# thomasdeppisch/eMagLS

Measured on AMD Instinct MI355X. Metric: eMagLS filter sets/s (N=4, 2702 dirs, 512 taps), higher is better.
Workload: dtype f64; 1 GPU; BASELINE config 3: getEMagLsFilters em32 r=4.2cm N=4 complex-SH, 2702 dirs, 512 taps, 48 kHz; one filter set per step, inputs resident in HBM; dirs=2702, taps=512, sim_order=19, bins=512, k_cut=43, designs_resident_per_gpu=128, designs_per_batch=32, batches_in_flight=4, distinct_hrir_sets_resident=20, parallelism=independent jobs per GPU, one RCCL gather

## Files before the change

emagls_amd/csrc/args.hpp:

```cpp
#pragma once
#include "common.hpp"

namespace emagls {

struct FactorArgs {
    int S;
    int C;
    int ldS;
    int kb0;
    int P;
    const void* Tn;
    const cplx* bn;
    int nOrders;
    int bn_stride;
    const cplx* Xd;
    int64_t xd_stride;
    int reg_mode;
    double reg_c;
    double tol_dim;
    cplx* Z;
    cplx* Vws;
    double* sv;
    const cplx* Hq;
    int64_t ldHq;
// ... 50 lines not shown
    long long* timing;
    int fetch_mode;
    long long wait_ticks;
    int force_global;
    const double* dir_azi;
    const double* dir_zen;
    const double* mic_azi;
    const double* mic_zen;
    const int* smap;
    const cplx* bsc;
    int nord_pad;
    int synth_split;
    int synth_prio;
    const cplx* Winit;
    cplx* U;
};
constexpr int SWEEP_MULTI_MAX = 16;
struct HalfSweepMulti {
    int n;
    HalfSweepArgs a[SWEEP_MULTI_MAX];
};
constexpr int REG_SWEEP_MAX = 32;


}
```

emagls_amd/csrc/batch_run.hip:

```cpp
#include "host_internal.hpp"

void emagls_batch_forget(emagls_batch* b, emagls_plan* p) {
    for (auto& q : b->plans) if (q == p) q = nullptr;
}

namespace {
void batch_sweep_stage(emagls_batch& b) {
    const int nb = (int)b.plans.size();
    std::vector<HalfSweepArgs> ha((size_t)nb);
    for (int j = 0; j < nb; ++j) ha[j] = emagls_half_args(*b.plans[j]);
    if (b.atf_share || b.geo_share)
        for (int j = 1; j < nb; ++j) {
            ha[j].G = ha[0].G; ha[j].Yri = ha[0].Yri; ha[j].Mw = ha[0].Mw; ha[j].cond_ok = ha[0].cond_ok;
            ha[j].bsc = ha[0].bsc; ha[j].smap = ha[0].smap;
            ha[j].skip_flag = ha[0].skip_flag;
        }
    const bool reg = b.plans[0]->sweep_persist && reg_sweep_wanted(b.plans.data(), nb);
    for (auto* q : b.plans) q->reg_sweep = reg;
    if (!reg && nb > SWEEP_MULTI_MAX) throw Error(EMAGLS_ERR_UNSUPPORTED, "internal: more than 16 designs in a batch need the register-resident sweep");
    HalfSweepMulti h{};
    h.n = std::min(nb, SWEEP_MULTI_MAX);
    for (int j = 0; j < h.n; ++j) h.a[j] = ha[j];
    emagls_plan& q0 = *b.plans[0];
    const int kk0 = std::max(q0.kcut0, 1);
    if (kk0 >= q0.P) return;
    if (q0.sweep_persist) {
        hipStream_t ss = b.stream;
        {
            SweepGate gate(ss, reg ? reg_sweep_gate_cost((int)q0.D, nb) : 0);
            if (b.lanes) { BatchScope sc(nb, b.stride); launch_zero(q0.get("ll"), q0.bufs["ll"].bytes, ss); }
            else for (auto* q : b.plans) launch_zero(q->get("ll"), q->bufs["ll"].bytes, ss);
            if (reg) {
// ... 289 lines not shown
            };
            if (hh_end > 1) {
                bc("Yc", 0, g.bufs["Yc"].bytes);
                bc(cb ? "R" : "Rc", 0, g.bufs[cb ? "R" : "Rc"].bytes);
                bc("Vws", 0, sizeof(cplx) * (size_t)(hh_end - 1) * g.C * ldSh);
                bc("Nw", 0, sizeof(cplx) * (size_t)(hh_end - 1) * g.C * g.C);
                bc("tauw", 0, sizeof(double) * (size_t)(hh_end - 1) * g.C);
                bc("cond_ok", 0, sizeof(double) * (size_t)g.P);
            }
            if (gf > 0 && gf < ls_end) {
                bc("G", (size_t)(gf - g.g0) * g_stride_b, (size_t)(ls_end - gf) * g_stride_b);
                bc("Mw", 0, sizeof(cplx) * (size_t)ls_end * g.C * g.C);
            }
        }
        if (b.geo_ls_shared) geo_yls_stage(b, b.stream);
        hrir_side(1);
    } else if (b.lanes) {
        BatchScope sc(n, b.stride);
        Scoped from(p0.geo_from, &p0);
        emagls_post_sweep(p0);
    } else {
        for (auto* p : b.plans) {
            Scoped from(p->geo_from, &p0);
            emagls_post_sweep(*p);
        }
    }
}
void batch_execute_geo(emagls_batch& b) {
    const bool warm = batch_geo_next_is_warm(b);
    if (!warm) {
        b.geo_kept_version = ~0ull;
        b.geo_ran_version = batch_geo_version(b);
        b.geo_cold_pending = true;
        if (b.geo_ls_shared) {
            const emagls_plan& p0 = *b.plans[0];
            const int ls_end = std::min(p0.kcut0, p0.P), hh_ls = std::min(p0.hh_end, ls_end);
            const void *y0 = b.yls.get(), *z0 = b.zls.get();
            b.yls.grow(sizeof(cplx) * (size_t)(ls_end - 1) * p0.C * p0.ldD);
            b.zls.grow(sizeof(cplx) * (size_t)std::max(hh_ls, 1) * p0.C * p0.ldS_h);
            if (b.yls.get() != y0 || b.zls.get() != z0) { b.group[0].reset(); b.warm.reset(); }
        }
    }
    batch_run_two_graphs(b, warm ? b.warm : b.group[0], batch_geo_stage, warm ? 1 : 0, sweep_launch_count(*b.plans[0]));
    b.last_form = warm ? 2 : 1;
    ++(warm ? b.geo_warm_runs : b.geo_cold_runs);
}

void batch_magls_decide_sharing(emagls_batch& b, bool sweep_needed) {
    bool share = false;
    emagls_plan& p0 = *b.plans[0];
    if (b.geo_want && b.plans.size() > 1 && !p0.custom_basis && !p0.diffuse && (p0.sweep_persist || !sweep_needed)) {
        share = batch_inputs_same(b, {"hrir_azi", "hrir_zen"}, b.geo_checked_version, b.geo_inputs_same);
        for (auto* p : b.plans) share = share && !p->custom_basis && p->d.fs == p0.d.fs;
    }
    batch_set_sharing(b, b.geo_share, share);
// ... 287 lines not shown
```

emagls_amd/csrc/capi.hip:

```cpp
#include "host_internal.hpp"

namespace {

struct CachedPlan {
    std::unique_ptr<emagls_plan> plan;
    emagls_design_desc desc{};
    int device = 0;
    bool busy = false;
    uint64_t last_use = 0;
};
std::mutex g_cache_mu;
std::vector<CachedPlan> g_cache;
uint64_t g_cache_tick = 0;

int one_shot(const emagls_design_desc& desc, const double* hL, const double* hR, const double* azi, const double* zen,
             const double* mic_azi, const double* mic_zen, const double* atf, const double* atf_azi, const double* atf_zen,
             void* wL, void* wR, double* mean_dev, const void* Y_hrir = nullptr, const void* Y_mic = nullptr) {
    return guarded([&] {
        int dev = 0;
        HIP_CHECK(hipGetDevice(&dev));
        emagls_plan* p = nullptr;
        std::unique_ptr<emagls_plan> fresh;
        bool cached = false;
        {
// ... 436 lines not shown
    return guarded([&] {
        DeviceGuard dg(p ? p->device : -1);
        if (!p || !name || !nbytes) throw Error(EMAGLS_ERR_ARG, "null pointer");
        if (std::string(name) == "Yls") {
            emagls_batch* b = p->owner;
            if (!b || !b->geo_share || !b->geo_ls_shared || !b->yls.get()) throw Error(EMAGLS_ERR_ARG, "Yls: the plan's batch keeps no such operand");
            const emagls_plan& p0 = *b->plans[0];
            const size_t bytes = sizeof(cplx) * (size_t)(std::min(p0.kcut0, p0.P) - 1) * p0.C * p0.ldD;
            if (!dst) { *nbytes = bytes; return; }
            HIP_CHECK(hipStreamSynchronize(b->stream));
            const size_t n = std::min(*nbytes, bytes);
            HIP_CHECK(hipMemcpy(dst, b->yls.get(), n, hipMemcpyDeviceToHost));
            *nbytes = n;
            return;
        }
        auto it = p->bufs.find(name);
        if (it == p->bufs.end()) throw Error(EMAGLS_ERR_ARG, std::string("unknown buffer ") + name);
        if (!dst) { *nbytes = it->second.bytes; return; }
        HIP_CHECK(hipStreamSynchronize(p->stream));
        const size_t n = std::min(*nbytes, it->second.bytes);
        HIP_CHECK(hipMemcpy(dst, it->second.p, n, hipMemcpyDeviceToHost));
        *nbytes = n;
    });
}
void* emagls_plan_stream(emagls_plan* p) { return p ? (void*)p->stream : nullptr; }

int emagls_batch_create(emagls_plan** plans, int nplans, emagls_batch** batch) {
    return guarded([&] {
        if (!plans || !batch || nplans < 1) throw Error(EMAGLS_ERR_ARG, "invalid argument");
        const int batch_max = std::max(g_batch_max.load(), g_batch_max_override);
// ... 387 lines not shown
```

emagls_amd/csrc/device_mem.hpp:

```cpp
#pragma once
#include <hipfft/hipfft.h>

#include <algorithm>
#include <deque>

#include "kernels.hpp"

namespace emagls {

struct DevMem {
    DevMem() = default;
    explicit DevMem(size_t bytes) { alloc(bytes); }
    DevMem(DevMem&& o) noexcept : p_(o.p_), cap_(o.cap_) { o.p_ = nullptr; o.cap_ = 0; }
    DevMem& operator=(DevMem&& o) noexcept {
        if (this != &o) { reset(); p_ = o.p_; cap_ = o.cap_; o.p_ = nullptr; o.cap_ = 0; }
        return *this;
    }
    ~DevMem() { reset(); }
    void reset() {
        if (p_) (void)hipFree(p_);
        p_ = nullptr; cap_ = 0;
    }
    void alloc(size_t bytes) {
        reset();
        HIP_CHECK(hipMalloc(&p_, bytes));
        cap_ = bytes;
    }
    void grow(size_t bytes) {
        bytes = std::max<size_t>(bytes, 16);
        if (bytes > cap_) alloc(bytes);
    }
    template <typename T = void> T* get() const { return static_cast<T*>(p_); }
    size_t capacity() const { return cap_; }

private:
    void* p_ = nullptr;
    size_t cap_ = 0;
};

struct FftPlan {
    FftPlan() = default;
    FftPlan(FftPlan&& o) noexcept : h_(o.h_) { o.h_ = 0; }
    FftPlan& operator=(FftPlan&& o) noexcept {
        if (this != &o) { reset(); h_ = o.h_; o.h_ = 0; }
        return *this;
// ... 40 lines not shown
```

emagls_amd/csrc/host_internal.hpp:

```cpp
#pragma once
#include <atomic>
#include <chrono>
#include <cstdlib>
#include <cstring>
#include <deque>
#include <map>
#include <memory>
#include <mutex>
#include <shared_mutex>
#include <string>
#include <thread>
#include <utility>
#include <vector>

#include "../../include/emagls.h"
#include "array_model.hpp"
#include "device_mem.hpp"
#include "kernels.hpp"

using namespace emagls;

struct emagls_batch;
void emagls_batch_forget(emagls_batch* b, emagls_plan* p);

// ... 328 lines not shown
    hipStream_t stream = nullptr;
    bool own_stream = true;
    bool atf = false, atf_share = false, atf_inputs_same = false;
    uint64_t atf_checked_version = ~0ull;
    bool magls = false;
    bool geo_want = false, geo_share = false, geo_inputs_same = false;
    uint64_t geo_checked_version = ~0ull;
    uint64_t geo_kept_version = ~0ull;
    uint64_t geo_ran_version = ~0ull;
    bool geo_cold_pending = false;
    CapturedGraph warm;
    int last_form = 0;
    long long geo_cold_runs = 0, geo_warm_runs = 0;
    bool geo_ls_shared = false;
    emagls::DevMem yls, zls;
    emagls::DevMem cmp_flag;
    int nstreams = 1;
    hipStream_t side[3] = {nullptr, nullptr, nullptr};
    CapturedGraph group[4];
    int prof_level = 0;
    hipEvent_t sweep_ev[2] = {nullptr, nullptr};
    CapturedGraph post;
    bool side0_external = false;
    int order_hint = 0;
    int groups = 1;
    CapturedGraph group_hh[4];
    hipStream_t hh_stream[4] = {nullptr, nullptr, nullptr, nullptr};
    bool defer_hh = false;
    bool alone = true;
    int eager_runs = 0;
// ... 108 lines not shown
```

emagls_amd/csrc/kernels.hpp:

```cpp
#pragma once
#include <algorithm>
#include <functional>

#include "common.hpp"

namespace emagls {

void launch_zero(void* p, size_t bytes, hipStream_t st);
void launch_compare_words(const void* a, const void* b, size_t bytes, int* differ, hipStream_t st);
void launch_broadcast_lanes(const void* src, size_t bytes, size_t stride, int nlanes, hipStream_t st);
struct LanePtrs { void* p[64]; };
void launch_scatter_lanes(const void* srcL, const void* srcR, size_t stride, size_t bytes, int n, const LanePtrs& dst, hipStream_t st);
void launch_gather_buffers(const LanePtrs& src, const LanePtrs& dst, int nbuf, size_t bytes, hipStream_t st);
struct BufferMoves { const void* src[96]; void* dst[96]; size_t bytes[96]; int n; };
void launch_move_buffers(const BufferMoves& m, hipStream_t st);
void launch_ch_basis(int N, int M, const double* azi, bool cplx_basis, void* out, int ld, hipStream_t st, bool out_real = false);
void launch_sh_coeff(int N, double* tab, hipStream_t st);
inline size_t esz(bool c) { return c ? sizeof(cplx) : sizeof(double); }
inline size_t sh_coeff_count(int N) { return (size_t)2 * (N + 1) * (N + 1) + 2 * (N + 1); }
void launch_sh_basis(int N, int64_t D, const double* azi, const double* zen, const double* tab, bool cplx_basis,
                     void* Y, int64_t ld, hipStream_t st);
void launch_transpose_conj(const void* Y, int64_t D, int64_t S, int64_t ldY, void* Yt, int64_t Dpad, int64_t ldYt,
                           bool is_cplx, bool conj_it, hipStream_t st);

// ... 79 lines not shown
void launch_sweep_synth(const HalfSweepMulti& m, hipStream_t st);
void launch_yls_gram(const void* bsc, int nord_pad, const double* dir_azi, const double* dir_zen, const double* mic_azi, const double* mic_zen,
                     const int* smap, const double* Pm, const void* Mw, int D, int nOut, int kb_lo, int kb_hi, void* Yls, int64_t ldD, hipStream_t st);
void launch_ls_shared_rows(const void* Hc, int64_t ldH, int ls_end, const void* Yls, int64_t ldD, int D, int C, int P, void* W, hipStream_t st);
void synth_cosines_debug(const double* dir_azi, const double* dir_zen, int64_t ndirs, const double* mic_azi, const double* mic_zen, int nmics, double* x2);
void synth_operand_debug(const void* bsc, int nbins, int nord_pad, const double* x, int64_t nx, int gs, void* g_plus, void* g_minus);
int reg_sweep_max_units();
bool reg_sweep_supported(int D, int nmics, int nunits, int nOrd);
size_t reg_sweep_ll_bytes(int D, int nmics);
int reg_sweep_capacity(int D);
int reg_sweep_slots_per_xcd();
int reg_sweep_pick_waves(int D, int ndesigns);
int reg_sweep_gate_cost(int D, int ndesigns);
bool reg_sweep_fits(int D, int nmics, int nunits, int nOrd, int ndesigns);
void launch_sweep_reg(const HalfSweepArgs* args_dev, const HalfSweepArgs& a0, int n, hipStream_t st);
double reg_contract_selftest();
double gram_tile_selftest(bool four);
void store_sweep_args(const HalfSweepArgs* host, int n, HalfSweepArgs* dev, hipStream_t st);
void launch_sweep_finalize(const void* Wpart, void* W, int nWG, int C, int P, int kb_last, hipStream_t st);
void launch_hy_conj(const void* Hc, int64_t ldD, int nrows, const void* Yc, int64_t ldY, bool y_cplx, int D, int S, void* Pw, void* out,
                    int ldS, hipStream_t st);
size_t hy_workspace_elems(int nrows, int ldS);
void launch_ypinv(const void* Q, int64_t ldQ, bool q_cplx, const void* Zb, int ldS, int D, int S, int C, void* Ypinv,
                  int64_t ldD, hipStream_t st);
void launch_ls_apply(const void* Hc, int64_t ldH, int n_c, const void* Zf, bool z_cplx, int64_t ldD, int D, int C, int P,
                     int kb_lo, int kb_hi, void* W, hipStream_t st);
void launch_ls_filters(const double* hL, const double* hR, int64_t L, int D, const void* Yp, bool cplx_basis, int64_t ldD,
                       int C, void* wL, void* wR, hipStream_t st);
void launch_conj_copy(const void* in, void* out, int64_t n, bool is_cplx, hipStream_t st);
void launch_sh_rows_to_complex(void* W, int C, int nrows, int order, hipStream_t st);
// ... 201 lines not shown
```

emagls_amd/csrc/sweep_reg.hip:

```cpp
#include "device_mem.hpp"
#include "persist_common.hpp"
#include "synth_common.hpp"

#include <algorithm>
#include <map>
#include <mutex>

namespace emagls {

namespace {

constexpr int RG_MLD = 36;

constexpr int DPP_ROR4 = 0x124, DPP_ROR8 = 0x128;
__device__ __forceinline__ int rg_slot_set(int i, int x) { return i < 4 ? 0 : i < 8 ? 1 : x >> 1; }
__device__ __forceinline__ int rg_slot_unit(int i, int x) { return i < 8 ? 4 * (i & 3) + x : 16 + (x & 1); }

template <int NUL>
__device__ __forceinline__ void rg_contract(const cplx (&E)[NUL], const cplx (&O)[NUL], const cplx (&ts)[2], int lane, bool slot8, double* wp) {
    static_assert(NUL == 9, "quad layout of 18 units");
    const int x = lane & 3;
    double ar[2], ai[2];
#pragma unroll
    for (int s = 0; s < 2; ++s) { ar[s] = (x & 1) ? ts[s].y : ts[s].x; ai[s] = (x & 1) ? -ts[s].x : ts[s].y; }
// ... 86 lines not shown
__device__ __forceinline__ void gll_put(gu64_t dst, u64 word, bool local) {
    if (local) __hip_atomic_store(dst, word, __ATOMIC_RELAXED, __HIP_MEMORY_SCOPE_WORKGROUP);
    else __hip_atomic_store(dst, word, __ATOMIC_RELAXED, __HIP_MEMORY_SCOPE_AGENT);
}
__device__ __forceinline__ void gll_load16_async(u32x4_t& out, gu64_t p) { asm volatile("global_load_dwordx4 %0, %1, off sc1" : "=v"(out) : "v"(p) : "memory"); }

constexpr int RG_POLL = 12;
__device__ __forceinline__ void rg_wait_loads(u32x4_t (&g)[RG_POLL]) {
    asm volatile("s_waitcnt vmcnt(0)" : "+v"(g[0]), "+v"(g[1]), "+v"(g[2]), "+v"(g[3]), "+v"(g[4]), "+v"(g[5]), "+v"(g[6]), "+v"(g[7]), "+v"(g[8]), "+v"(g[9]),
                 "+v"(g[10]), "+v"(g[11]) :: "memory");
}
constexpr int RG_NUL = 9;
constexpr int RG_NEX = 4 * PS_CMAX;
constexpr int RG_SVC = 256;

template <int NUL, int NW>
__global__ void __launch_bounds__(64 * NW) __attribute__((amdgpu_waves_per_eu(3))) sweep_reg_kernel(const HalfSweepArgs* __restrict__ args, int n, int nWG, int spread, int prio) {
    constexpr int NT = 64 * NW, DPW = 32 * NW;
    constexpr int NU2 = 2 * NUL;
    constexpr int NVW = 8 * NU2;
    constexpr int GA = (NUL + 1) / 2, GB = NUL - GA;
    static_assert(GB >= 1 && NW % 2 == 0 && NT >= RG_SVC, "layout");
    extern __shared__ __attribute__((aligned(16))) char dyn[];
    cplx* ring = reinterpret_cast<cplx*>(dyn);
    cplx* ms = ring + 2 * SY_NORD;
    cplx* WE = ms + PS_CMAX * RG_MLD;
    cplx* WO = WE + 2 * NU2;
    double* vt = reinterpret_cast<double*>(WO + 2 * NU2);
    double* wpart = vt + 2 * RG_NEX;
    double* xs = wpart + NW * NVW;
    __shared__ int s_abort, s_local;

    int design, member;
    if (spread) {
        design = (int)blockIdx.x / nWG;
        member = (int)blockIdx.x - design * nWG;
    } else {
        const int xcd = blockIdx.x & 7, rest = blockIdx.x >> 3;
        const int sub = rest / nWG;
        member = rest - sub * nWG;
// ... 11 lines not shown
    const gcc_t bsc = RG_GLOBAL(const cplx, a.bsc);
    const gcd_t Winit = RG_GLOBAL(const double, a.Winit);
    cplx __attribute__((address_space(1)))* const Uout = RG_GLOBAL(cplx, a.U);
    long long* const timing = a.timing;
    int* const abort_flag = a.abort_flag;
    const long long wait_ticks = a.wait_ticks;
    const int* smap = a.smap;
    const int npr = smap[32], nsg = smap[33], nun = npr + nsg;
    const gu64_t part_ll = RG_GLOBAL(u64, a.ll);
    const gu64_t xcc_ll = part_ll + (size_t)2 * nWG * RG_NEX * 2;
    if (tid == 0) { s_abort = 0; s_local = 0; }
    const int d0 = member * DPW;
    auto dir_of = [&](int t, int s) __attribute__((always_inline)) { return d0 + 32 * (t >> 6) + 16 * s + ((t & 63) >> 2); };

    {
        const size_t ncplx = (size_t)2 * SY_NORD + PS_CMAX * RG_MLD + 4 * NU2;
        for (size_t i = tid; i < ncplx; i += NT) ring[i] = mk(0, 0);
        for (int i = tid; i < 2 * RG_NEX + NW * NVW; i += NT) vt[i] = 0.0;
        double sd[2], cd[2], daz[2];
#pragma unroll
        for (int s = 0; s < 2; ++s) {
            const int dgi = dir_of(tid, s) < D ? dir_of(tid, s) : D - 1;
            synth_zen(a.dir_zen[dgi], sd[s], cd[s]);
            daz[s] = a.dir_azi[dgi];
        }
#pragma unroll 1
        for (int i = 0; i < NUL; ++i) {
            const int u = rg_slot_unit(i, tid & 3), s = rg_slot_set(i, tid & 3);
            double v = 0.0;
            if (u < nun) {
                const int jm = smap[u < npr ? 2 * u : 2 * npr + (u - npr)];
                double sm, cm;
                synth_zen(a.mic_zen ? a.mic_zen[jm] : 1.5707963267948966, sm, cm);
                v = synth_x2(s ? sd[1] : sd[0], s ? cd[1] : cd[0], sm, cm, (s ? daz[1] : daz[0]) - a.mic_azi[jm]);
            }
            xs[i * NT + tid] = v;
        }
    }
    __syncthreads();

    if (tid < nord_pad) {
        ring[(kfirst & 1) * SY_NORD + tid] = ldg(bsc + (int64_t)kfirst * nord_pad + tid);
        const int k1 = kfirst + 1 < P ? kfirst + 1 : P - 1;
        ring[((kfirst + 1) & 1) * SY_NORD + tid] = ldg(bsc + (int64_t)k1 * nord_pad + tid);
    }
    constexpr int NLM = 4;
    cplx mReg[NLM];
    auto fetch_m = [&](int kbm, int t) __attribute__((always_inline)) {
        const int r = t >> 3, c0 = (t & 7) * 4;
        const gcc_t M = Mw + (int64_t)kbm * C * C + r * C + c0;
#pragma unroll
        for (int i = 0; i < NLM; ++i) mReg[i] = ldg(M + i);
    };
    auto stage_m = [&](int t) __attribute__((always_inline)) {
        const int r = t >> 3, c0 = (t & 7) * 4;
#pragma unroll
// ... 15 lines not shown
        const unsigned tag0 = 0x58434300u;
        if (lane == 0) gll_put(xcc_ll + member, ((u64)tag0 << 32) | xcc, false);
        bool alive = true, same = true;
        for (int base = 0; base < nWG && alive; base += 64) {
            u64 w = 0;
            alive = ll_wait([&] {
                if (base + lane >= nWG) return true;
                w = gll_load(xcc_ll + base + lane);
                return ll_ok(w, tag0);
            }, abort_flag, wait_ticks);
            same = same && __builtin_amdgcn_ballot_w64(base + lane < nWG && (unsigned)w != xcc) == 0;
        }
        if (lane == 0) {
            s_local = alive && same && a.force_global == 0;
            if (!alive) s_abort = 1;
            if (timing && member == 1) timing[15] = s_local;
        }
    }
    __syncthreads();
    const bool local = s_local != 0;
    if (s_abort) return;

    const bool slot8 = nun > 16 || GB < 2;
    cplx E[NUL], O[NUL];
#pragma unroll
    for (int u = 0; u < NUL; ++u) { E[u] = mk(0, 0); O[u] = mk(0, 0); }

#define RSTAMP(i) do { if (timing && member == 1 && tid == 0 && kb < P) timing[(int64_t)kb * 16 + (i)] = (long long)wall_clock64(); } while (0)
    for (int kb = kfirst; kb <= P; ++kb) {
        const bool first = (kb == kfirst);
        const bool last = (kb == P);
        const bool nyq = (kb == P - 1);
        RSTAMP(7);
        if (!last) {
            const cplx* bs = ring + (kb & 1) * SY_NORD;
            const double* xcol = xs + launder(tid);
            synth_units<0, GA, NUL, NT>(xcol, E, O, bs, nord_pad);
            __builtin_amdgcn_sched_barrier(0);
            if (slot8) synth_units<GA, GB, NUL, NT>(xcol, E, O, bs, nord_pad);
            else synth_units<GA, GB - 1, NUL, NT>(xcol, E, O, bs, nord_pad);
            __builtin_amdgcn_sched_barrier(0);
        }
        RSTAMP(0);
        if (launder(tid) < RG_SVC) {
            const int t = launder(tid);
            const int j = t & (RG_NEX - 1), half = t >> 7;
            if (first) {
                vt[t] = half == 0 ? Winit[j] : 0.0;
            } else {
// ... 45 lines not shown
                if (c < 2 * npr) {
                    if ((c & 1) == 0) { WE[e * NU2 + (c >> 1)] = acc + other; WO[e * NU2 + (c >> 1)] = acc - other; }
                } else {
                    WE[e * NU2 + npr + (c - 2 * npr)] = acc; WO[e * NU2 + npr + (c - 2 * npr)] = acc;
                }
                if (member == 0 && !first) {
                    cplx __attribute__((address_space(1)))* dst = Uout + ((int64_t)e * P + (kb - 1)) * PS_CMAX + c;
                    const cplx v = vc[c] + vc[RG_NEX / 2 + c];
                    dst->x = v.x; dst->y = v.y;
                }
            }
        }
        if (last) break;
        __syncthreads();
        RSTAMP(3);
        const bool svc = launder(tid) < RG_SVC;
        if (svc) fetch_m(kb, launder(tid));
        cplx ts[2];
        {
            const int t = launder(tid);
            const int x = t & 3;
            cplx p[2][2];
#pragma unroll
            for (int s = 0; s < 2; ++s) { p[s][0] = mk(0, 0); p[s][1] = mk(0, 0); }
#pragma unroll
            for (int r = 0; r < 4; ++r) {
                const int u = 4 * r + x;
                const cplx we0 = WE[u], wo0 = WO[u], we1 = WE[NU2 + u], wo1 = WO[NU2 + u];
#pragma unroll
                for (int s = 0; s < 2; ++s) {
// ... 16 lines not shown
#pragma unroll
            for (int s = 0; s < 2; ++s) {
                const cplx pe0 = group_sum<4>(p[s][0]), pe1 = group_sum<4>(p[s][1]);
                const cplx pe = (x & 2) ? pe1 : pe0;
                ts[s] = dir_of(t, s) < D ? unit_phase(hCur[s], pe, nyq) : mk(0, 0);
            }
        }
        __builtin_amdgcn_sched_barrier(0);
        {
            const int t = launder(tid);
            rg_contract<NUL>(E, O, ts, t & 63, slot8, wpart + (t >> 6) * NVW);
        }
        {
            const int t = launder(tid);
            fetch_h(kb + 1, hNext, t);
            if (t < nord_pad) ring[(kb & 1) * SY_NORD + t] = ldg(bsc + (int64_t)(kb + 2 < P ? kb + 2 : P - 1) * nord_pad + t);
        }
        __syncthreads();
        RSTAMP(4);
        if (launder(tid) < RG_NEX) {
            const int t = launder(tid);
            const int xe = t >> 6, xr = (t >> 1) & 31, xri = t & 1;
            double v = 0.0;
            if (xr < C) {
                const int xu = xr < 2 * npr ? (xr >> 1) : npr + (xr - 2 * npr);
                const bool xneg = xr < 2 * npr && (xr & 1);
                const double* wE = wpart + 8 * xu + 2 * xe + xri;
                double sE = 0.0, sO = 0.0;
#pragma unroll
                for (int w = 0; w < NW; ++w) { sE += wE[w * NVW]; sO += wE[w * NVW + 4]; }
                v = xneg ? sE - sO : sE + sO;
// ... 21 lines not shown
#pragma unroll
    for (int s = 0; s < 2; ++s) ts[s] = ldc(t + (16 * s + (lane >> 2)) * 2 + (x >> 1));
    rg_contract<RG_NUL>(E, O, ts, lane, true, out);
}

__global__ void __launch_bounds__(64) store_args_kernel(HalfSweepMulti m, HalfSweepArgs* dst) {
    const int nw = (int)(sizeof(HalfSweepArgs) / 8);
    for (int j = 0; j < m.n; ++j) {
        const unsigned long long* src = reinterpret_cast<const unsigned long long*>(&m.a[j]);
        unsigned long long* d = reinterpret_cast<unsigned long long*>(dst + j);
        for (int i = threadIdx.x; i < nw; i += 64) d[i] = src[i];
    }
}
static_assert(sizeof(HalfSweepArgs) % 8 == 0, "argument block in whole words");

size_t reg_dyn_bytes(int nul, int nw) {
    const size_t nu2 = 2 * (size_t)nul, nvw = 8 * nu2;
    return sizeof(cplx) * ((size_t)2 * SY_NORD + PS_CMAX * RG_MLD + 4 * nu2) +
           sizeof(double) * (2 * RG_NEX + (size_t)nw * nvw + (size_t)nul * 64 * nw);
}
constexpr int RG_WAVES[] = {4, 6, 8, 10, 12};
const void* reg_kernel_ptr(int nw) {
    switch (nw) {
        case 4: return reinterpret_cast<const void*>(sweep_reg_kernel<RG_NUL, 4>);
        case 6: return reinterpret_cast<const void*>(sweep_reg_kernel<RG_NUL, 6>);
        case 8: return reinterpret_cast<const void*>(sweep_reg_kernel<RG_NUL, 8>);
        case 10: return reinterpret_cast<const void*>(sweep_reg_kernel<RG_NUL, 10>);
        default: return reinterpret_cast<const void*>(sweep_reg_kernel<RG_NUL, 12>);
    }
}
void reg_set_attributes() {
    static PerDeviceOnce attr_once;
    if (attr_once.first())
        for (int nw : RG_WAVES) HIP_CHECK(hipFuncSetAttribute(reg_kernel_ptr(nw), hipFuncAttributeMaxDynamicSharedMemorySize, 150 * 1024));
}
int reg_nwg(int D, int nw) { return (int)ceil_div(D, 32 * nw); }
int reg_occupancy(int nw) {
    static std::mutex mu;
    static std::map<std::pair<int, int>, int> cache;
    int dev = 0;
    HIP_CHECK(hipGetDevice(&dev));
    std::lock_guard<std::mutex> lk(mu);
    auto it = cache.find({dev, nw});
    if (it != cache.end()) return it->second;
    reg_set_attributes();
    int nb = 0;
    if (hipOccupancyMaxActiveBlocksPerMultiprocessor(&nb, reg_kernel_ptr(nw), 64 * nw, reg_dyn_bytes(RG_NUL, nw)) != hipSuccess) { (void)hipGetLastError(); nb = 0; }
    cache[{dev, nw}] = nb;
    return nb;
}
int reg_wg_cost(int nw) { return nw == 4 ? 1 : 3; }

}

int reg_sweep_max_units() { return 2 * RG_NUL; }
bool reg_sweep_supported(int D, int nmics, int nunits, int nOrd) {
    return nmics >= 2 && nmics <= PS_CMAX && nunits >= 1 && nunits <= 2 * RG_NUL && D >= 1 && reg_nwg(D, 12) <= 32 && nOrd <= SY_NORD;
}
size_t reg_sweep_ll_bytes(int D, int nmics) {
    const size_t nwg = (size_t)reg_nwg(D, 4);
    (void)nmics;
    return sizeof(u64) * ((size_t)2 * nwg * RG_NEX * 2 + nwg + 64);
}
// ... 17 lines not shown
}
int reg_sweep_gate_cost(int D, int ndesigns) {
    if (const int ns = reg_sweep_spread_waves(D, ndesigns)) return (int)ceil_div((int64_t)ndesigns * reg_nwg(D, ns), 8) * reg_wg_cost(ns);
    const int nw = reg_sweep_pick_waves(D, ndesigns);
    return nw ? (int)ceil_div(ndesigns, 8) * reg_nwg(D, nw) * reg_wg_cost(nw) : 0;
}
int reg_sweep_capacity(int D) {
    int n = 0;
    for (int k = 8; k <= REG_SWEEP_MAX; k += 8) if (reg_sweep_pick_waves(D, k)) n = k;
    return n;
}
bool reg_sweep_fits(int D, int nmics, int nunits, int nOrd, int ndesigns) {
    return reg_sweep_supported(D, nmics, nunits, nOrd) && reg_sweep_pick_waves(D, ndesigns) != 0;
}

void launch_sweep_reg(const HalfSweepArgs* args_dev, const HalfSweepArgs& a0, int n, hipStream_t st) {
    const int ns = reg_sweep_spread_waves(a0.D, n);
    const int nw = ns ? ns : reg_sweep_pick_waves(a0.D, n);
    if (!nw) throw Error(2, "register-resident sweep: the launch cannot be resident");
    const int nWG = reg_nwg(a0.D, nw), spread = ns ? 1 : 0;
    const unsigned nblocks = spread ? (unsigned)(n * nWG) : 8u * (unsigned)nWG * (unsigned)ceil_div(n, 8);
    const size_t dyn = reg_dyn_bytes(RG_NUL, nw);
    reg_set_attributes();
    const int prio = sw_int<Sw::REG_PRIO>();
    switch (nw) {
        case 4: sweep_reg_kernel<RG_NUL, 4><<<dim3(nblocks), 256, dyn, st>>>(args_dev, n, nWG, spread, prio); break;
        case 6: sweep_reg_kernel<RG_NUL, 6><<<dim3(nblocks), 384, dyn, st>>>(args_dev, n, nWG, spread, prio); break;
        case 8: sweep_reg_kernel<RG_NUL, 8><<<dim3(nblocks), 512, dyn, st>>>(args_dev, n, nWG, spread, prio); break;
        case 10: sweep_reg_kernel<RG_NUL, 10><<<dim3(nblocks), 640, dyn, st>>>(args_dev, n, nWG, spread, prio); break;
        default: sweep_reg_kernel<RG_NUL, 12><<<dim3(nblocks), 768, dyn, st>>>(args_dev, n, nWG, spread, prio); break;
    }
    KERNEL_CHECK();
}

double reg_contract_selftest() {
    constexpr int ND = 32, NU = 2 * RG_NUL, NO = 8 * NU;
    cplx h_t[ND * 2], h_g[ND * NU * 2];
    double h_out[NO], want[NO] = {0};
    unsigned long long x = 88172645463325252ull;
    auto rnd = [&] { x ^= x << 13; x ^= x >> 7; x ^= x << 17; return (double)(x % 2000001ull) / 1000000.0 - 1.0; };
    for (cplx& v : h_t) { v.x = rnd(); v.y = rnd(); }
    for (cplx& v : h_g) { v.x = rnd(); v.y = rnd(); }
    for (int d = 0; d < ND; ++d)
        for (int u = 0; u < NU; ++u)
            for (int eo = 0; eo < 2; ++eo)
                for (int e = 0; e < 2; ++e) {
// ... 30 lines not shown
```

emagls_amd/csrc/switches.hpp:

```cpp
#pragma once
#include <climits>
#include <cmath>

namespace emagls {

#define EMAGLS_SWITCHES(X) \
    X(PLAN_CACHE,        INT,  4,     0, INT_MAX,   PROCESS, "shapes the one-shot entry points keep alive (0 = off)") \
    X(BATCH_MAX,         INT,  8,     1, 32,        PROCESS, "initial limit of designs per batch, read at load time (emagls_set_batch_max changes it at run time; the job scheduler sets it per chunk)") \
    X(BATCH_GROUPS,      INT,  2,     1, 4,         CALL,    "lane groups of a batch of more than 8 designs before its sweep (1 = one launch sequence)") \
    X(BATCH_LANES,       ON0,  1,     0, 1,         CALL,    "=0: batches in stream mode (per-plan pipelines) instead of lane mode") \
    X(DEBUG_LANES,       ON1,  0,     0, 1,         CALL,    "=1: why a batch was refused lane mode or common routes, on stderr") \
    X(STAGGER,           ON0,  1,     0, 1,         PROCESS, "=0: both lane groups of a batch issue the stages before the sweep in one order (default: complementary orders)") \
    X(DEFER_HH,          INT,  1,     0, 2,         PROCESS, "the orthonormal route of the low bins next to the sweep: 0 never, 1 batches and designs that have the device to themselves, 2 every lane batch") \
    X(GEO_KEEP,          ON0,  1,     0, 1,         PROCESS, "=0: sharing batches run their geometry stages on every execute") \
    X(GEO_LS_SHARED,     ON0,  1,     0, 1,         CALL,    "=0: sharing batches carry every HRIR set's least-squares rows through the factors instead of one kept Y_reg_inv per bin") \
    X(GRAM_LDS,          ON0,  1,     0, 1,         PROCESS, "=0: lane batches take the K-split Gram kernel + reduce instead of the LDS-staged one") \
    X(GRAM_MFMA4,        ON1,  0,     0, 1,         CALL,    "=1: the Gram tile on the 4 x 4 x 4 MFMA shape (measured slower; the tests' second form)") \
    X(XCD_RUNS,          ON0,  1,     0, 1,         PROCESS, "=0: gram_lds, gemm_tn_f64, synth_ls take their tiles in dispatch order instead of XCD-aware runs") \
    X(GRAM_ROUTE,        ON0,  1,     0, 1,         CALL,    "=0: no Gram route (all bins Householder + Jacobi)") \
    X(GRAM_COND_EST,     REAL, 3e3,   -HUGE_VAL, HUGE_VAL, CALL, "conditioning estimate below which the Gram route starts (the device check stays at 3e4)") \
    X(JACOBI_RUN,        INT,  0,     1, INT_MAX,   PROCESS, "bins per Jacobi workgroup on the Gram route (0: single bins where the stages are forked, runs of 2 in lane groups)") \
    X(REAL_INTERNAL,     ON0,  1,     0, 1,         CALL,    "=0: complex-basis eMagLS / eMagLS2 designs on the complex-arithmetic pipeline") \
    X(NO_GRAPH,          ON1,  0,     0, 1,         CALL,    "=1: eager launches instead of hipGraph replay (plans and batches, when they are created)") \
    X(STREAMS,           INT,  0,     1, 4,         CALL,    "streams of a single plan (0: one, until emagls_plan_set_streams)") \
    X(ONESHOT_STREAMS,   INT,  1,     1, 3,         CALL,    "streams of the one-shot plans of array designs") \
    X(SWEEP_PERSIST,     ON0,  1,     0, 1,         CALL,    "=0: launch-per-bin sweep instead of the persistent one") \
    X(PERSIST_GLOBAL,    ON1,  0,     0, 1,         CALL,    "=1: write-through granules even when a design sits on one XCD") \
    X(SWEEP_SYNTH,       ON0,  1,     0, 1,         CALL,    "=0: array designs on materialised operands instead of the synthesising sweep (when a plan is created)") \
    X(SWEEP_TWIN,        ON0,  1,     0, 1,         CALL,    "=0: launches of 9-16 designs as two independent workgroups per CU instead of twin workgroups") \
    X(SWEEP_REG,         INT,  1,     0, 2,         CALL,    "register-resident sweep: 0 never (the slab form), 1 for launches of more than 8 designs, 2 always") \
// ... 56 lines not shown
```

Before: 4290 filter sets/s.

## Precompute register-sweep synthesis operand once per shared geometry and load it

Adds a kernel that evaluates the sweep's synthesised operand (E/O per unit, per bin and direction group) into a device table kept per sharing geometry. The register-resident sweep kernel gains a KEPT variant that prefetches this operand from global memory for the next bin instead of recomputing it from direction/mic angles and the bsc ring in every launch. This removes repeated synthesis arithmetic and frees LDS (ring and xs), in exchange for extra HBM traffic and a table that can reach hundreds of MB. The table is built only on cold geometry runs and is gated by a size limit and an occupancy check.

```diff
diff --git a/emagls_amd/csrc/args.hpp b/emagls_amd/csrc/args.hpp
--- a/emagls_amd/csrc/args.hpp
+++ b/emagls_amd/csrc/args.hpp
@@ -88,6 +88,7 @@
     int synth_prio;
     const cplx* Winit;
     cplx* U;
+    const cplx* opnd;
 };
 constexpr int SWEEP_MULTI_MAX = 16;
 struct HalfSweepMulti {
diff --git a/emagls_amd/csrc/batch_run.hip b/emagls_amd/csrc/batch_run.hip
--- a/emagls_amd/csrc/batch_run.hip
+++ b/emagls_amd/csrc/batch_run.hip
@@ -16,6 +16,8 @@
             ha[j].skip_flag = ha[0].skip_flag;
         }
     const bool reg = b.plans[0]->sweep_persist && reg_sweep_wanted(b.plans.data(), nb);
+    if (reg && b.geo_share && b.sweep_opnd_on)
+        for (int j = 0; j < nb; ++j) ha[j].opnd = b.sweep_opnd.get<const cplx>();
     for (auto* q : b.plans) q->reg_sweep = reg;
     if (!reg && nb > SWEEP_MULTI_MAX) throw Error(EMAGLS_ERR_UNSUPPORTED, "internal: more than 16 designs in a batch need the register-resident sweep");
     HalfSweepMulti h{};
@@ -335,6 +337,7 @@
             }
         }
         if (b.geo_ls_shared) geo_yls_stage(b, b.stream);
+        if (b.sweep_opnd_on) launch_reg_operand(emagls_half_args(p0), b.sweep_opnd.get(), b.stream);
         hrir_side(1);
     } else if (b.lanes) {
         BatchScope sc(n, b.stride);
@@ -360,6 +363,22 @@
             b.yls.grow(sizeof(cplx) * (size_t)(ls_end - 1) * p0.C * p0.ldD);
             b.zls.grow(sizeof(cplx) * (size_t)std::max(hh_ls, 1) * p0.C * p0.ldS_h);
             if (b.yls.get() != y0 || b.zls.get() != z0) { b.group[0].reset(); b.warm.reset(); }
+        }
+        {
+            emagls_plan& p0 = *b.plans[0];
+            const int kk0 = std::max(p0.kcut0, 1);
+            const size_t bytes = reg_operand_bytes((int)p0.D, p0.P, kk0);
+            const bool want = p0.synth && p0.sweep_persist && bytes > 0 && bytes <= (size_t)sw_int<Sw::GEO_SWEEP_OPERAND_MB>() * 1048576 &&
+                              reg_sweep_wanted(b.plans.data(), (int)b.plans.size()) && reg_sweep_reads_kept((int)p0.D, (int)b.plans.size());
+            const void* t0 = b.sweep_opnd.get();
+            const bool was = b.sweep_opnd_on;
+            if (want) {
+                if (bytes > b.sweep_opnd.capacity()) HIP_CHECK(hipStreamSynchronize(b.stream));
+                b.sweep_opnd_on = b.sweep_opnd.try_grow(bytes);
+            } else {
+                b.sweep_opnd_on = false;
+            }
+            if (b.sweep_opnd.get() != t0 || b.sweep_opnd_on != was) { b.group[0].reset(); b.warm.reset(); }
         }
     }
     batch_run_two_graphs(b, warm ? b.warm : b.group[0], batch_geo_stage, warm ? 1 : 0, sweep_launch_count(*b.plans[0]));
diff --git a/emagls_amd/csrc/capi.hip b/emagls_amd/csrc/capi.hip
--- a/emagls_amd/csrc/capi.hip
+++ b/emagls_amd/csrc/capi.hip
@@ -474,6 +474,18 @@
             *nbytes = n;
             return;
         }
+        if (std::string(name) == "SweepOperand") {
+            emagls_batch* b = p->owner;
+            if (!b || !b->geo_share || !b->sweep_opnd_on || !b->sweep_opnd.get()) throw Error(EMAGLS_ERR_ARG, "SweepOperand: the plan's batch keeps no such operand");
+            const emagls_plan& p0 = *b->plans[0];
+            const size_t bytes = reg_operand_bytes((int)p0.D, p0.P, std::max(p0.kcut0, 1));
+            if (!dst) { *nbytes = bytes; return; }
+            HIP_CHECK(hipStreamSynchronize(b->stream));
+            const size_t n = std::min(*nbytes, bytes);
+            HIP_CHECK(hipMemcpy(dst, b->sweep_opnd.get(), n, hipMemcpyDeviceToHost));
+            *nbytes = n;
+            return;
+        }
         auto it = p->bufs.find(name);
         if (it == p->bufs.end()) throw Error(EMAGLS_ERR_ARG, std::string("unknown buffer ") + name);
         if (!dst) { *nbytes = it->second.bytes; return; }
diff --git a/emagls_amd/csrc/device_mem.hpp b/emagls_amd/csrc/device_mem.hpp
--- a/emagls_amd/csrc/device_mem.hpp
+++ b/emagls_amd/csrc/device_mem.hpp
@@ -29,6 +29,14 @@
     void grow(size_t bytes) {
         bytes = std::max<size_t>(bytes, 16);
         if (bytes > cap_) alloc(bytes);
+    }
+    bool try_grow(size_t bytes) {
+        bytes = std::max<size_t>(bytes, 16);
+        if (bytes <= cap_) return true;
+        reset();
+        if (hipMalloc(&p_, bytes) != hipSuccess) { (void)hipGetLastError(); p_ = nullptr; return false; }
+        cap_ = bytes;
+        return true;
     }
     template <typename T = void> T* get() const { return static_cast<T*>(p_); }
     size_t capacity() const { return cap_; }
diff --git a/emagls_amd/csrc/host_internal.hpp b/emagls_amd/csrc/host_internal.hpp
--- a/emagls_amd/csrc/host_internal.hpp
+++ b/emagls_amd/csrc/host_internal.hpp
@@ -366,6 +366,8 @@
     long long geo_cold_runs = 0, geo_warm_runs = 0;
     bool geo_ls_shared = false;
     emagls::DevMem yls, zls;
+    emagls::DevMem sweep_opnd;
+    bool sweep_opnd_on = false;
     emagls::DevMem cmp_flag;
     int nstreams = 1;
     hipStream_t side[3] = {nullptr, nullptr, nullptr};
diff --git a/emagls_amd/csrc/kernels.hpp b/emagls_amd/csrc/kernels.hpp
--- a/emagls_amd/csrc/kernels.hpp
+++ b/emagls_amd/csrc/kernels.hpp
@@ -117,6 +117,9 @@
 int reg_sweep_gate_cost(int D, int ndesigns);
 bool reg_sweep_fits(int D, int nmics, int nunits, int nOrd, int ndesigns);
 void launch_sweep_reg(const HalfSweepArgs* args_dev, const HalfSweepArgs& a0, int n, hipStream_t st);
+bool reg_sweep_reads_kept(int D, int ndesigns);
+size_t reg_operand_bytes(int D, int P, int kfirst);
+void launch_reg_operand(const HalfSweepArgs& a0, void* table, hipStream_t st);
 double reg_contract_selftest();
 double gram_tile_selftest(bool four);
 void store_sweep_args(const HalfSweepArgs* host, int n, HalfSweepArgs* dev, hipStream_t st);
diff --git a/emagls_amd/csrc/sweep_reg.hip b/emagls_amd/csrc/sweep_reg.hip
--- a/emagls_amd/csrc/sweep_reg.hip
+++ b/emagls_amd/csrc/sweep_reg.hip
@@ -5,6 +5,7 @@
 #include <algorithm>
 #include <map>
 #include <mutex>
+#include <tuple>
 
 namespace emagls {
 
@@ -124,7 +125,67 @@
 constexpr int RG_NEX = 4 * PS_CMAX;
 constexpr int RG_SVC = 256;
 
-template <int NUL, int NW>
+template <int NUL>
+__device__ __forceinline__ void rg_fill_xs(const HalfSweepArgs& a, int dir0, int dir1, int x, double* xs, int stride, int col) {
+    const int* smap = a.smap;
+    const int npr = smap[32], nun = npr + smap[33];
+    double sd[2], cd[2], daz[2];
+#pragma unroll
+    for (int s = 0; s < 2; ++s) {
+        const int dgi = min(s ? dir1 : dir0, a.D - 1);
+        synth_zen(a.dir_zen[dgi], sd[s], cd[s]);
+        daz[s] = a.dir_azi[dgi];
+    }
+#pragma unroll 1
+    for (int i = 0; i < NUL; ++i) {
+        const int u = rg_slot_unit(i, x), s = rg_slot_set(i, x);
+        double v = 0.0;
+        if (u < nun) {
+            const int jm = smap[u < npr ? 2 * u : 2 * npr + (u - npr)];
+            double sm, cm;
+            synth_zen(a.mic_zen ? a.mic_zen[jm] : 1.5707963267948966, sm, cm);
+            v = synth_x2(s ? sd[1] : sd[0], s ? cd[1] : cd[0], sm, cm, (s ? daz[1] : daz[0]) - a.mic_azi[jm]);
+        }
+        xs[i * stride + col] = v;
+    }
+}
+
+constexpr int RG_OPW = 4;
+__device__ __forceinline__ int64_t rg_operand_index(int kbrel, int ngw, int gw, int nul, int lane) { return (((int64_t)kbrel * ngw + gw) * (2 * nul)) * 64 + lane; }
+template <int NUL>
+__global__ void __launch_bounds__(64 * RG_OPW) reg_operand_kernel(HalfSweepArgs a, cplx* __restrict__ table, int ngw) {
+    constexpr int NT = 64 * RG_OPW;
+    constexpr int GA = (NUL + 1) / 2, GB = NUL - GA;
+    __shared__ __attribute__((aligned(16))) cplx ring[SY_NORD];
+    __shared__ double xs[NUL * NT];
+    const int tid = threadIdx.x, lane = tid & 63;
+    const int gw = (int)blockIdx.x * RG_OPW + (tid >> 6);
+    const int nord_pad = a.nord_pad;
+    const int nun = a.smap[32] + a.smap[33];
+    const bool slot8 = nun > 16 || GB < 2;
+    rg_fill_xs<NUL>(a, 32 * gw + (lane >> 2), 32 * gw + 16 + (lane >> 2), tid & 3, xs, NT, tid);
+    for (int kb = a.kfirst + (int)blockIdx.y; kb < a.P; kb += (int)gridDim.y) {
+        __syncthreads();
+        if (tid < nord_pad) ring[tid] = ldc(a.bsc + (int64_t)kb * nord_pad + tid);
+        __syncthreads();
+        cplx E[NUL], O[NUL];
+#pragma unroll
+        for (int u = 0; u < NUL; ++u) { E[u] = mk(0, 0); O[u] = mk(0, 0); }
+        const double* xcol = xs + tid;
+        synth_units<0, GA, NUL, NT>(xcol, E, O, ring, nord_pad);
+        __builtin_amdgcn_sched_barrier(0);
+        if (slot8) synth_units<GA, GB, NUL, NT>(xcol, E, O, ring, nord_pad);
+        else synth_units<GA, GB - 1, NUL, NT>(xcol, E, O, ring, nord_pad);
+        __builtin_amdgcn_sched_barrier(0);
+        if (gw < ngw) {
+            cplx* dst = table + rg_operand_index(kb - a.kfirst, ngw, gw, NUL, lane);
+#pragma unroll
+            for (int i = 0; i < NUL; ++i) { dst[(2 * i) * 64] = E[i]; dst[(2 * i + 1) * 64] = O[i]; }
+        }
+    }
+}
+
+template <int NUL, int NW, bool KEPT>
 __global__ void __launch_bounds__(64 * NW) __attribute__((amdgpu_waves_per_eu(3))) sweep_reg_kernel(const HalfSweepArgs* __restrict__ args, int n, int nWG, int spread, int prio) {
     constexpr int NT = 64 * NW, DPW = 32 * NW;
     constexpr int NU2 = 2 * NUL;
@@ -132,8 +193,9 @@
     constexpr int GA = (NUL + 1) / 2, GB = NUL - GA;
     static_assert(GB >= 1 && NW % 2 == 0 && NT >= RG_SVC, "layout");
     extern __shared__ __attribute__((aligned(16))) char dyn[];
+    constexpr int NRING = KEPT ? 0 : 2 * SY_NORD;
     cplx* ring = reinterpret_cast<cplx*>(dyn);
-    cplx* ms = ring + 2 * SY_NORD;
+    cplx* ms = ring + NRING;
     cplx* WE = ms + PS_CMAX * RG_MLD;
     cplx* WO = WE + 2 * NU2;
     double* vt = reinterpret_cast<double*>(WO + 2 * NU2);
@@ -175,32 +237,14 @@
     auto dir_of = [&](int t, int s) __attribute__((always_inline)) { return d0 + 32 * (t >> 6) + 16 * s + ((t & 63) >> 2); };
 
     {
-        const size_t ncplx = (size_t)2 * SY_NORD + PS_CMAX * RG_MLD + 4 * NU2;
+        const size_t ncplx = (size_t)NRING + PS_CMAX * RG_MLD + 4 * NU2;
         for (size_t i = tid; i < ncplx; i += NT) ring[i] = mk(0, 0);
         for (int i = tid; i < 2 * RG_NEX + NW * NVW; i += NT) vt[i] = 0.0;
-        double sd[2], cd[2], daz[2];
-#pragma unroll
-        for (int s = 0; s < 2; ++s) {
-            const int dgi = dir_of(tid, s) < D ? dir_of(tid, s) : D - 1;
-            synth_zen(a.dir_zen[dgi], sd[s], cd[s]);
-            daz[s] = a.dir_azi[dgi];
-        }
-#pragma unroll 1
-        for (int i = 0; i < NUL; ++i) {
-            const int u = rg_slot_unit(i, tid & 3), s = rg_slot_set(i, tid & 3);
-            double v = 0.0;
-            if (u < nun) {
-                const int jm = smap[u < npr ? 2 * u : 2 * npr + (u - npr)];
-                double sm, cm;
-                synth_zen(a.mic_zen ? a.mic_zen[jm] : 1.5707963267948966, sm, cm);
-                v = synth_x2(s ? sd[1] : sd[0], s ? cd[1] : cd[0], sm, cm, (s ? daz[1] : daz[0]) - a.mic_azi[jm]);
-            }
-            xs[i * NT + tid] = v;
-        }
+        if constexpr (!KEPT) rg_fill_xs<NUL>(a, dir_of(tid, 0), dir_of(tid, 1), tid & 3, xs, NT, tid);
     }
     __syncthreads();
 
-    if (tid < nord_pad) {
+    if (!KEPT && tid < nord_pad) {
         ring[(kfirst & 1) * SY_NORD + tid] = ldg(bsc + (int64_t)kfirst * nord_pad + tid);
         const int k1 = kfirst + 1 < P ? kfirst + 1 : P - 1;
         ring[((kfirst + 1) & 1) * SY_NORD + tid] = ldg(bsc + (int64_t)k1 * nord_pad + tid);
@@ -246,7 +290,7 @@
         if (lane == 0) {
             s_local = alive && same && a.force_global == 0;
             if (!alive) s_abort = 1;
-            if (timing && member == 1) timing[15] = s_local;
+            if (timing && member == 1) { timing[15] = s_local; timing[14] = KEPT ? 1 : 0; }
         }
     }
     __syncthreads();
@@ -257,6 +301,28 @@
     cplx E[NUL], O[NUL];
 #pragma unroll
     for (int u = 0; u < NUL; ++u) { E[u] = mk(0, 0); O[u] = mk(0, 0); }
+
+    const gcc_t opnd = RG_GLOBAL(const cplx, a.opnd);
+    const int ngw = (D + 31) >> 5;
+    auto fetch_operand = [&](int kb, int t) __attribute__((always_inline)) {
+        const int gw = min((d0 >> 5) + (t >> 6), ngw - 1);
+        const gcc_t src = opnd + rg_operand_index(kb - kfirst, ngw, gw, NUL, t & 63);
+#pragma unroll
+        for (int i = 0; i < NUL; ++i) {
+            if (i == NUL - 1 && !slot8) break;
+            E[i] = ldg(src + (2 * i) * 64); O[i] = ldg(src + (2 * i + 1) * 64);
+        }
+    };
+    auto await_operand = [&]() __attribute__((always_inline)) {
+        asm volatile("s_waitcnt vmcnt(0)" : "+v"(E[0].x), "+v"(E[0].y), "+v"(E[1].x), "+v"(E[1].y), "+v"(E[2].x), "+v"(E[2].y), "+v"(E[3].x), "+v"(E[3].y), "+v"(E[4].x),
+                     "+v"(E[4].y), "+v"(E[5].x), "+v"(E[5].y), "+v"(E[6].x), "+v"(E[6].y), "+v"(E[7].x), "+v"(E[7].y), "+v"(E[8].x), "+v"(E[8].y) :: "memory");
+        asm volatile("" : "+v"(O[0].x), "+v"(O[0].y), "+v"(O[1].x), "+v"(O[1].y), "+v"(O[2].x), "+v"(O[2].y), "+v"(O[3].x), "+v"(O[3].y), "+v"(O[4].x),
+                     "+v"(O[4].y), "+v"(O[5].x), "+v"(O[5].y), "+v"(O[6].x), "+v"(O[6].y), "+v"(O[7].x), "+v"(O[7].y), "+v"(O[8].x), "+v"(O[8].y) :: "memory");
+    };
+    if constexpr (KEPT) {
+        static_assert(NUL == 9, "await_operand names nine slots");
+        fetch_operand(kfirst, tid);
+    }
 
 #define RSTAMP(i) do { if (timing && member == 1 && tid == 0 && kb < P) timing[(int64_t)kb * 16 + (i)] = (long long)wall_clock64(); } while (0)
     for (int kb = kfirst; kb <= P; ++kb) {
@@ -264,7 +330,7 @@
         const bool last = (kb == P);
         const bool nyq = (kb == P - 1);
         RSTAMP(7);
-        if (!last) {
+        if constexpr (!KEPT) if (!last) {
             const cplx* bs = ring + (kb & 1) * SY_NORD;
             const double* xcol = xs + launder(tid);
             synth_units<0, GA, NUL, NT>(xcol, E, O, bs, nord_pad);
@@ -340,6 +406,7 @@
         if (last) break;
         __syncthreads();
         RSTAMP(3);
+        if constexpr (KEPT) { await_operand(); RSTAMP(9); }
         const bool svc = launder(tid) < RG_SVC;
         if (svc) fetch_m(kb, launder(tid));
         cplx ts[2];
@@ -386,7 +453,8 @@
         {
             const int t = launder(tid);
             fetch_h(kb + 1, hNext, t);
-            if (t < nord_pad) ring[(kb & 1) * SY_NORD + t] = ldg(bsc + (int64_t)(kb + 2 < P ? kb + 2 : P - 1) * nord_pad + t);
+            if constexpr (KEPT) { if (kb + 1 < P) fetch_operand(kb + 1, t); }
+            else if (t < nord_pad) ring[(kb & 1) * SY_NORD + t] = ldg(bsc + (int64_t)(kb + 2 < P ? kb + 2 : P - 1) * nord_pad + t);
         }
         __syncthreads();
         RSTAMP(4);
@@ -438,39 +506,43 @@
 }
 static_assert(sizeof(HalfSweepArgs) % 8 == 0, "argument block in whole words");
 
-size_t reg_dyn_bytes(int nul, int nw) {
+size_t reg_dyn_bytes(int nul, int nw, bool kept) {
     const size_t nu2 = 2 * (size_t)nul, nvw = 8 * nu2;
-    return sizeof(cplx) * ((size_t)2 * SY_NORD + PS_CMAX * RG_MLD + 4 * nu2) +
-           sizeof(double) * (2 * RG_NEX + (size_t)nw * nvw + (size_t)nul * 64 * nw);
+    return sizeof(cplx) * ((kept ? 0 : (size_t)2 * SY_NORD) + PS_CMAX * RG_MLD + 4 * nu2) +
+           sizeof(double) * (2 * RG_NEX + (size_t)nw * nvw + (kept ? 0 : (size_t)nul * 64 * nw));
 }
 constexpr int RG_WAVES[] = {4, 6, 8, 10, 12};
-const void* reg_kernel_ptr(int nw) {
+typedef void (*reg_kernel_t)(const HalfSweepArgs*, int, int, int, int);
+template <bool KEPT> reg_kernel_t reg_kernel_of(int nw) {
     switch (nw) {
-        case 4: return reinterpret_cast<const void*>(sweep_reg_kernel<RG_NUL, 4>);
-        case 6: return reinterpret_cast<const void*>(sweep_reg_kernel<RG_NUL, 6>);
-        case 8: return reinterpret_cast<const void*>(sweep_reg_kernel<RG_NUL, 8>);
-        case 10: return reinterpret_cast<const void*>(sweep_reg_kernel<RG_NUL, 10>);
-        default: return reinterpret_cast<const void*>(sweep_reg_kernel<RG_NUL, 12>);
-    }
-}
+        case 4: return sweep_reg_kernel<RG_NUL, 4, KEPT>;
+        case 6: return sweep_reg_kernel<RG_NUL, 6, KEPT>;
+        case 8: return sweep_reg_kernel<RG_NUL, 8, KEPT>;
+        case 10: return sweep_reg_kernel<RG_NUL, 10, KEPT>;
+        default: return sweep_reg_kernel<RG_NUL, 12, KEPT>;
+    }
+}
+reg_kernel_t reg_kernel_fn(int nw, bool kept) { return kept ? reg_kernel_of<true>(nw) : reg_kernel_of<false>(nw); }
+const void* reg_kernel_ptr(int nw, bool kept) { return reinterpret_cast<const void*>(reg_kernel_fn(nw, kept)); }
 void reg_set_attributes() {
     static PerDeviceOnce attr_once;
     if (attr_once.first())
-        for (int nw : RG_WAVES) HIP_CHECK(hipFuncSetAttribute(reg_kernel_ptr(nw), hipFuncAttributeMaxDynamicSharedMemorySize, 150 * 1024));
+        for (int nw : RG_WAVES)
+            for (bool kept : {false, true}) HIP_CHECK(hipFuncSetAttribute(reg_kernel_ptr(nw, kept), hipFuncAttributeMaxDynamicSharedMemorySize, 150 * 1024));
 }
 int reg_nwg(int D, int nw) { return (int)ceil_div(D, 32 * nw); }
-int reg_occupancy(int nw) {
+int reg_occupancy(int nw, bool kept = false) {
     static std::mutex mu;
-    static std::map<std::pair<int, int>, int> cache;
+    static std::map<std::tuple<int, int, bool>, int> cache;
     int dev = 0;
     HIP_CHECK(hipGetDevice(&dev));
     std::lock_guard<std::mutex> lk(mu);
-    auto it = cache.find({dev, nw});
+    auto it = cache.find({dev, nw, kept});
     if (it != cache.end()) return it->second;
     reg_set_attributes();
     int nb = 0;
-    if (hipOccupancyMaxActiveBlocksPerMultiprocessor(&nb, reg_kernel_ptr(nw), 64 * nw, reg_dyn_bytes(RG_NUL, nw)) != hipSuccess) { (void)hipGetLastError(); nb = 0; }
-    cache[{dev, nw}] = nb;
+    if (hipOccupancyMaxActiveBlocksPerMultiprocessor(&nb, reg_kernel_ptr(nw, kept), 64 * nw, reg_dyn_bytes(RG_NUL, nw, kept)) != hipSuccess) { (void)hipGetLastError(); nb = 0; }
+    cache[{dev, nw, kept}] = nb;
     return nb;
 }
 int reg_wg_cost(int nw) { return nw == 4 ? 1 : 3; }
@@ -518,22 +590,34 @@
     return reg_sweep_supported(D, nmics, nunits, nOrd) && reg_sweep_pick_waves(D, ndesigns) != 0;
 }
 
+bool reg_sweep_reads_kept(int D, int n) {
+    const int mode = sw_int<Sw::GEO_SWEEP_OPERAND>();
+    const int ns = reg_sweep_spread_waves(D, n);
+    const int nw = ns ? ns : reg_sweep_pick_waves(D, n);
+    return mode != 0 && nw != 0 && (mode == 2 || ns == 0) && reg_occupancy(nw, true) >= reg_occupancy(nw, false);
+}
+
 void launch_sweep_reg(const HalfSweepArgs* args_dev, const HalfSweepArgs& a0, int n, hipStream_t st) {
     const int ns = reg_sweep_spread_waves(a0.D, n);
     const int nw = ns ? ns : reg_sweep_pick_waves(a0.D, n);
     if (!nw) throw Error(2, "register-resident sweep: the launch cannot be resident");
     const int nWG = reg_nwg(a0.D, nw), spread = ns ? 1 : 0;
     const unsigned nblocks = spread ? (unsigned)(n * nWG) : 8u * (unsigned)nWG * (unsigned)ceil_div(n, 8);
-    const size_t dyn = reg_dyn_bytes(RG_NUL, nw);
+    const bool kept = a0.opnd != nullptr && reg_sweep_reads_kept(a0.D, n);
+    const size_t dyn = reg_dyn_bytes(RG_NUL, nw, kept);
     reg_set_attributes();
     const int prio = sw_int<Sw::REG_PRIO>();
-    switch (nw) {
-        case 4: sweep_reg_kernel<RG_NUL, 4><<<dim3(nblocks), 256, dyn, st>>>(args_dev, n, nWG, spread, prio); break;
-        case 6: sweep_reg_kernel<RG_NUL, 6><<<dim3(nblocks), 384, dyn, st>>>(args_dev, n, nWG, spread, prio); break;
-        case 8: sweep_reg_kernel<RG_NUL, 8><<<dim3(nblocks), 512, dyn, st>>>(args_dev, n, nWG, spread, prio); break;
-        case 10: sweep_reg_kernel<RG_NUL, 10><<<dim3(nblocks), 640, dyn, st>>>(args_dev, n, nWG, spread, prio); break;
-        default: sweep_reg_kernel<RG_NUL, 12><<<dim3(nblocks), 768, dyn, st>>>(args_dev, n, nWG, spread, prio); break;
-    }
+    reg_kernel_fn(nw, kept)<<<dim3(nblocks), 64 * nw, dyn, st>>>(args_dev, n, nWG, spread, prio);
+    KERNEL_CHECK();
+}
+
+size_t reg_operand_bytes(int D, int P, int kfirst) {
+    return P > kfirst ? sizeof(cplx) * (size_t)(P - kfirst) * (size_t)ceil_div(D, 32) * (2 * RG_NUL) * 64 : 0;
+}
+void launch_reg_operand(const HalfSweepArgs& a0, void* table, hipStream_t st) {
+    const int ngw = (int)ceil_div(a0.D, 32), nbins = a0.P - a0.kfirst;
+    if (nbins < 1) return;
+    reg_operand_kernel<RG_NUL><<<dim3((unsigned)ceil_div(ngw, RG_OPW), (unsigned)std::min(nbins, 48)), 64 * RG_OPW, 0, st>>>(a0, static_cast<cplx*>(table), ngw);
     KERNEL_CHECK();
 }
 
diff --git a/emagls_amd/csrc/switches.hpp b/emagls_amd/csrc/switches.hpp
--- a/emagls_amd/csrc/switches.hpp
+++ b/emagls_amd/csrc/switches.hpp
@@ -14,6 +14,8 @@
     X(DEFER_HH,          INT,  1,     0, 2,         PROCESS, "the orthonormal route of the low bins next to the sweep: 0 never, 1 batches and designs that have the device to themselves, 2 every lane batch") \
     X(GEO_KEEP,          ON0,  1,     0, 1,         PROCESS, "=0: sharing batches run their geometry stages on every execute") \
     X(GEO_LS_SHARED,     ON0,  1,     0, 1,         CALL,    "=0: sharing batches carry every HRIR set's least-squares rows through the factors instead of one kept Y_reg_inv per bin") \
+    X(GEO_SWEEP_OPERAND, INT,  1,     0, 2,         CALL,    "the register-resident sweep of a sharing batch loads its operand from one table kept per geometry: 0 never (evaluated inside every launch), 1 launches whose designs each stay on one XCD, 2 spread launches too") \
+    X(GEO_SWEEP_OPERAND_MB, INT, 1024, 0, INT_MAX,  CALL,    "largest kept sweep operand of a sharing batch, in MB (a larger one is not kept: the sweep evaluates it)") \
     X(GRAM_LDS,          ON0,  1,     0, 1,         PROCESS, "=0: lane batches take the K-split Gram kernel + reduce instead of the LDS-staged one") \
     X(GRAM_MFMA4,        ON1,  0,     0, 1,         CALL,    "=1: the Gram tile on the 4 x 4 x 4 MFMA shape (measured slower; the tests' second form)") \
     X(XCD_RUNS,          ON0,  1,     0, 1,         PROCESS, "=0: gram_lds, gemm_tn_f64, synth_ls take their tiles in dispatch order instead of XCD-aware runs") \
```

Result: no change. 4304 filter sets/s (median of 4 runs) (+0.3%).
